# norlab-ulaval/norlab_icp_mapper

Hardware: AMD Instinct MI355X
Metric: ICP iterations/sec, 100k-pt scan vs 1M-pt map (higher is better)
Workload: dtype f32; 1 GPU; single synthetic 100000-pt scan vs 1000000-pt map, point-to-point ICP, KDTreeMatcher knn 1 maxDist 2.0 epsilon 0, TrimmedDist 0.85, fixed 20 iterations per registration; chain=p2p, scene=box+pillars sigma=0.01 seeds 42/43/44 (SURVEY.md 8d), parallelism=scan-sharded x1, map replicated

## Files before the change

### norlab_icp_mapper_amd/csrc/common.h

```cpp
#pragma once

#include <hip/hip_runtime.h>
#include <stdint.h>
#include <math.h>
#include <cstring>
#include <string>
#include <vector>
#include <unordered_map>
#include <mutex>
#include <map>
#include <cstdlib>
#include <shared_mutex>

#include "../../include/icpmi.h"

#define ICPMI_NV 32
#define ICPMI_MAX_OUTLIER 8
#define ICPMI_MAX_SMOOTH 16
#define ICPMI_SEL_BINS 2048
#ifndef ICPMI_S2_COPIES
#define ICPMI_S2_COPIES 8
#endif
#define ICPMI_S2_C0 4096
#define ICPMI_S2_F0 (ICPMI_S2_C0 + ICPMI_S2_COPIES * 256)
#ifndef ICPMI_S2_FCOPIES
#define ICPMI_S2_FCOPIES 1
#endif
#define ICPMI_S2_C1 (ICPMI_S2_F0 + ICPMI_S2_FCOPIES * 65536)
#define ICPMI_S2_F1 (ICPMI_S2_C1 + 256)
#define ICPMI_ACC_COPIES 2
#define ICPMI_ACC_MAX_ADDS 128
#define ICPMI_ACC_PAD 16
#define ICPMI_ACC_U64 (ICPMI_ACC_COPIES * ICPMI_NV * 2 * ICPMI_ACC_PAD)
#define ICPMI_ACC_IDX(copy, i, limb) ((((copy) * ICPMI_NV + (i)) * 2 + (limb)) * ICPMI_ACC_PAD)
#define ICPMI_ACC_FLAG (ICPMI_ACC_IDX(0, 0, 0) + 8)
#define ICPMI_S2_ACC (ICPMI_S2_F1 + 65536)
#define ICPMI_WIN_BINS 7
#ifndef ICPMI_WIN_COPIES
#define ICPMI_WIN_COPIES 8
#endif
#define ICPMI_WIN_PAD 16
#define ICPMI_WIN_HDR (ICPMI_WIN_COPIES * 3 * ICPMI_WIN_PAD)
#define ICPMI_WIN_U64 (ICPMI_WIN_HDR + ICPMI_WIN_PAD)
#define ICPMI_WIN_MAX_COUNT (1ll << 21)
#define ICPMI_S2_WIN (ICPMI_S2_ACC + 2 * ICPMI_ACC_U64)
#define ICPMI_SELHIST_WORDS (ICPMI_S2_WIN + 2 * ICPMI_WIN_U64)
#define ICPMI_S2_FIDX(b) ((((b) & 255u) << 8) | ((b) >> 8))

#define ICPMI_MAX_K 32

#ifdef __HIPCC__
typedef float icpmi_vf4 __attribute__((ext_vector_type(4)));
#ifdef ICPMI_NT_STREAMS
__device__ __forceinline__ float4 ld_stream(const float4* p) { const icpmi_vf4 v = __builtin_nontemporal_load(reinterpret_cast<const icpmi_vf4*>(p)); return make_float4(v.x, v.y, v.z, v.w); }
__device__ __forceinline__ float ld_stream(const float* p) { return __builtin_nontemporal_load(p); }
__device__ __forceinline__ int ld_stream(const int* p) { return __builtin_nontemporal_load(p); }
__device__ __forceinline__ void st_stream(float4* p, float4 v) { icpmi_vf4 w; w.x = v.x; w.y = v.y; w.z = v.z; w.w = v.w; __builtin_nontemporal_store(w, reinterpret_cast<icpmi_vf4*>(p)); }
__device__ __forceinline__ void st_stream(float* p, float v) { __builtin_nontemporal_store(v, p); }
__device__ __forceinline__ void st_stream(int* p, int v) { __builtin_nontemporal_store(v, p); }
#else
template <class T> __device__ __forceinline__ T ld_stream(const T* p) { return *p; }
template <class T> __device__ __forceinline__ void st_stream(T* p, T v) { *p = v; }
#endif

struct WaveRun { bool head; int rank; int len; int head_lane; };
__device__ __forceinline__ WaveRun wave_run(unsigned key, bool valid)
{
    const int lane = threadIdx.x & 63;
    const unsigned prev = (unsigned)__shfl_up((int)key, 1, 64);
    const bool pvalid = __shfl_up((int)valid, 1, 64) != 0;
    const bool head = valid && (lane == 0 || !pvalid || prev != key);
    const unsigned long long heads = __ballot(head);
    const unsigned long long valids = __ballot(valid);
    WaveRun r;
    r.head = head;
    const unsigned long long below = heads & ((lane == 63) ? ~0ull : ((2ull << lane) - 1ull));
    r.head_lane = below ? 63 - __clzll((long long)below) : lane;
    r.rank = lane - r.head_lane;
    const unsigned long long above = (lane == 63) ? 0ull : (heads & ~((2ull << lane) - 1ull));
// ... 25 lines not shown
struct BatchArgs {
    int nscan;
    int qstride;
    int n[ICPMI_MAX_BATCH];
};
struct BatchSrc { const float4* p[ICPMI_MAX_BATCH]; };
static inline BatchArgs batch_of_one(int64_t n) { BatchArgs b; memset(&b, 0, sizeof b); b.nscan = 1; b.n[0] = (int)n; return b; }

struct LoopCfg {
    int   k;
    float max_dist;
    float maxr2;
    float inv1e, err2;
    int   ring_max;
    int   minimizer;
    int   n_out;
    int   out_type[ICPMI_MAX_OUTLIER];
    float out_param[ICPMI_MAX_OUTLIER];
    int   out_iparam[ICPMI_MAX_OUTLIER];
    float out_param2[ICPMI_MAX_OUTLIER];
    float out_param3[ICPMI_MAX_OUTLIER];
    int   ext;
    int   force_4dof;
    int   force_2d;
    int   is_2d;
    int   max_iter;
    int   use_diff;
    float min_rot, min_trans;
    int   smooth;
    int   use_bound;
    float max_rot, max_trans;
    int   has_read_normals;
    int   sensor_noise;
    const float* read_scalar;
};

struct IcpState {
    float T_iter[16];
    int   iter;
    int   done;
    int   error;
    int   stop_reason;
    int   counter;
    int   hist_n;
    double hq[(ICPMI_MAX_SMOOTH + 1) * 4];
    double ht[(ICPMI_MAX_SMOOTH + 1) * 3];
    double hrot[ICPMI_MAX_SMOOTH + 1];
    double htr[ICPMI_MAX_SMOOTH + 1];
    double init_q[4];
    unsigned sel_prefix;
    unsigned sel_rank;
    unsigned n_valid;
    unsigned sel_prefix_l[3];
    unsigned sel_rank_l[3];
    float limits[ICPMI_MAX_OUTLIER];
    unsigned vt_valid;
    float vt_ratio;
    float robust_med;
    float robust_scale;
    long long pairs;
    double wsum;
    unsigned hard_count;
    unsigned ticket;
    unsigned long long hard_total;
    unsigned seq;
    unsigned long long dbg[24];
// ... 655 lines not shown
```

### norlab_icp_mapper_amd/csrc/loop.hip

```cpp
#include "common.h"
#include "solve.h"
#include <cstring>

namespace {

template <int PASS, int MODE = 0>
__global__ __launch_bounds__(256) void sel_hist_kernel(const float* __restrict__ d2, int64_t count,
                                                       const IcpState* __restrict__ st, unsigned* __restrict__ ghist, int nb_scale = 0)
{
    if (st->done) return;
    if (blockIdx.x == 0 && threadIdx.x == 0) nn_stamp_close(const_cast<IcpState*>(st));
    if (MODE != 0 && nb_scale != 0 && st->iter + 1 > nb_scale) return;
    if (MODE == 3 && st->iter != 0) return;
    __shared__ unsigned h[ICPMI_SEL_BINS];
    for (int b = threadIdx.x; b < ICPMI_SEL_BINS; b += 256) h[b] = 0;
    __syncthreads();
    const unsigned prefix = st->sel_prefix;
    const float med = MODE == 2 ? st->robust_med : 0.f;
    for (int64_t i = (int64_t)blockIdx.x * 256 + threadIdx.x; i < count; i += (int64_t)gridDim.x * 256) {
        float v = d2[i];
        if (MODE == 0 || MODE == 3) { if (!(v != INFINITY && v > 0.f)) continue; }
        else {
            if (v == INFINITY) continue;
            if (MODE == 2) v = fabsf(v - med);
// ... 505 lines not shown
                const float rz = fmaf(T[10], az, fmaf(T[6], ay, T[2] * ax));
                ax = rx; ay = ry; az = rz;
            }
            const float4 b = ref_normals[sidx];
            const float dot = fmaf(az, b.z, fmaf(ay, b.y, ax * b.x));
            w *= (dot > cosf(prm)) ? 1.f : 0.f;
        } else if (EXT && type == ICPMI_OUT_GENERICDESCRIPTOR) {
            const int ip = lc.out_iparam[f];
            const float v = (ip & ICPMI_GEN_SOURCE_READING) ? lc.read_scalar[qi] : ref_scalar[orig];
            w *= (ip & ICPMI_GEN_SOFT) ? v : ((ip & ICPMI_GEN_LARGER) ? (v > prm ? 1.f : 0.f) : (v < prm ? 1.f : 0.f));
        } else if (EXT && type == ICPMI_OUT_ROBUST) {
            const int ip = lc.out_iparam[f];
            const int se = (ip >> 4) & 15, fct = ip & 15;
            const float sc = se != ICPMI_SCALE_NONE ? st->robust_scale : 1.f;
            const float res = ((ip >> 8) & 15) == ICPMI_DIST_POINT2PLANE ? plane2 : d2;
            const float kk = se != ICPMI_SCALE_BERG ? prm : (fct == ICPMI_ROB_CAUCHY ? 4.3040f : fct == ICPMI_ROB_TUKEY ? 7.0589f : fct == ICPMI_ROB_HUBER ? 2.0138f : prm);
            const float e2 = res / (sc * sc);
            const float apx = lc.out_param3[f];
            float rw = robust_weight(fct, e2, kk);
            if (apx > 0.f && apx != INFINITY && e2 >= apx * apx) rw = 0.f;
            w *= rw;
        }
    }
    return w;
}

__host__ __device__ __forceinline__ int acc_threads(int k) { return k > 1 ? 1024 : 256; }
__host__ __device__ __forceinline__ int acc_blocks_dev(int64_t count, int cap, int bt = 256)
{
    const int64_t nb = (count + bt - 1) / bt;
    return (int)(nb < 1 ? 1 : (nb > cap ? cap : nb));
}

template <int MIN, bool FUSED, bool EXT, int BT = 256>
__global__ __launch_bounds__(BT) void accumulate_kernel(const float4* __restrict__ reading, BatchArgs ba, int acc_cap, LoopCfg lc,
                                                         IcpState* __restrict__ st, const float4* __restrict__ map,
                                                         const float4* __restrict__ normals,
                                                         const float4* __restrict__ read_normals,
                                                         const int* __restrict__ sidx, const float* __restrict__ d2a,
                                                         unsigned* __restrict__ hists,
                                                         int fused_slot, int is_median, float factor,
                                                         const float4* __restrict__ match_pt, const int* __restrict__ qindex,
                                                         const float* __restrict__ ref_scalar, const float4* __restrict__ pnm)
{
    const int n = ba.n[blockIdx.y];
    const int nbe = acc_blocks_dev((int64_t)n * lc.k, acc_cap, BT);
    if ((int)blockIdx.x >= nbe) return;
    {
        const size_t qo = (size_t)blockIdx.y * (size_t)ba.qstride;
        reading += qo; sidx += qo * lc.k; d2a += qo * lc.k;
        if (match_pt) match_pt += qo;
        if (qindex) qindex += qo;
        if (read_normals) read_normals += qo;
        hists += (size_t)blockIdx.y * ICPMI_SELHIST_WORDS;
        st += blockIdx.y;
    }
    const int64_t count = (int64_t)n * lc.k;
    const int64_t stride = (int64_t)nbe * BT;
    const int64_t gtid = (int64_t)blockIdx.x * BT + threadIdx.x;
#ifdef ICPMI_ACC_STRIDED
    const int64_t estep = stride;
    const int64_t e_first = gtid, e_end = count;
#else
    const int64_t estep = BT;
    const int wgc = (nbe & 7) == 0 ? (int)(blockIdx.x & 7) * (nbe >> 3) + (int)(blockIdx.x >> 3) : (int)blockIdx.x;
    const int64_t per_wg = (count + nbe - 1) / nbe;
    const int64_t e_first = (int64_t)wgc * per_wg + threadIdx.x;
    const int64_t e_end = ((int64_t)wgc + 1) * per_wg < count ? ((int64_t)wgc + 1) * per_wg : count;
#endif
    constexpr int PF = BT > 256 ? 3 : 2;
    float pd2[PF]; int ps[PF]; float4 pr[PF], pq[PF];
#pragma unroll
    for (int u = 0; u < PF; ++u) {
        const int64_t e = e_first + u * estep;
        const bool in = e < e_end;
        pd2[u] = in ? ld_stream(d2a + e) : INFINITY;
        ps[u] = in ? ld_stream(sidx + e) : -1;
        pr[u] = ld_stream(reading + (in ? (int)(e / lc.k) : 0));
        pq[u] = (match_pt && in) ? ld_stream(match_pt + e) : ((pnm && ps[u] >= 0) ? pnm[2 * (size_t)ps[u]] : make_float4(0.f, 0.f, 0.f, 0.f));
    }
    const unsigned cv = (FUSED && threadIdx.x < 256) ? hists[ICPMI_S2_C1 + threadIdx.x] : 0u;
    float4 pn[PF];
#pragma unroll
    for (int u = 0; u < PF; ++u)
        pn[u] = (MIN == ICPMI_MIN_POINT_TO_PLANE && ps[u] >= 0) ? (pnm ? pnm[2 * (size_t)ps[u] + 1] : normals[ps[u]]) : make_float4(0.f, 0.f, 0.f, 0.f);
    if (st->done) return;
    if (blockIdx.x == 0 && threadIdx.x == 0) nn_stamp_close(const_cast<IcpState*>(st));
    float fused_limit = 0.f;
    if (FUSED) {
        __shared__ unsigned shsel[16];
        unsigned bin, rem, total;
        block_find_rank_2tier<1>(cv, hists + ICPMI_S2_F1, false, 0.f, st->sel_rank_l[0], shsel, bin, rem, total);
        const float q = __uint_as_float((st->sel_prefix_l[0] << 16) | bin);
        fused_limit = is_median ? factor * q : q;
        if (blockIdx.x == 0 && threadIdx.x == 0) st->limits[fused_slot] = fused_limit;
        for (int64_t i = gtid; i < ICPMI_S2_COPIES * 256 + ICPMI_S2_FCOPIES * 65536; i += stride) hists[ICPMI_S2_C0 + i] = 0;
        if (lc.k > 1) for (int64_t i = gtid; i < 2 * ICPMI_WIN_U64; i += stride) hists[ICPMI_S2_WIN + i] = 0;
    }
    constexpr int NVAL = MIN == ICPMI_MIN_POINT_TO_PLANE ? 27 : (MIN == ICPMI_MIN_POINT_TO_POINT ? 16 : 0);
    double acc[NVAL > 0 ? NVAL : 1];
#pragma unroll
    for (int i = 0; i < (NVAL > 0 ? NVAL : 1); ++i) acc[i] = 0.0;
    double wsum = 0.0, cnt = 0.0;
    double b2d[3] = {0.0, 0.0, 0.0};
    const float* T = st->T_iter;
    auto pair = [&](int64_t e, float d2, int s, float4 r, float4 qkept, float4 nkept, bool have_n) {
        if (d2 == INFINITY) return;
        const int qi = (int)(e / lc.k);
        float w;
        if (EXT) {
            const float3 pe = xf_point(T, r.x, r.y, r.z, r.w);
            const float4 qe = (match_pt || (pnm && have_n)) ? qkept : (pnm ? pnm[2 * (size_t)s] : map[s]);
            float plane2 = 0.f;
            if (normals) {
                const float4 ne = have_n && MIN == ICPMI_MIN_POINT_TO_PLANE ? nkept : (pnm ? pnm[2 * (size_t)s + 1] : normals[s]);
                const float dx = pe.x - qe.x, dy = pe.y - qe.y, dz = pe.z - qe.z;
                const float dot = dx * ne.x + dy * ne.y + dz * ne.z;
                plane2 = dot * dot;
            }
            w = match_weight<true>(lc, st, d2, T, read_normals, qindex ? qindex[qi] : qi, normals, s, FUSED ? fused_slot : -1, fused_limit,
                                   ref_scalar, __float_as_int(qe.w), plane2);
        } else w = match_weight(lc, st, d2, T, read_normals, qindex ? qindex[qi] : qi, normals, s, FUSED ? fused_slot : -1, fused_limit);
        if (w == 0.f) return;
        wsum += w; cnt += 1.0;
        if (MIN == ICPMI_MIN_IDENTITY) return;
        const float3 p = xf_point(T, r.x, r.y, r.z, r.w);
        const float4 q = (match_pt || (pnm && have_n)) ? qkept : (pnm ? pnm[2 * (size_t)s] : map[s]);
        if (MIN == ICPMI_MIN_POINT_TO_POINT) {
// ... 36 lines not shown
    const int lane = threadIdx.x & 63, wv = threadIdx.x >> 6;
    double val[ICPMI_NV];
#pragma unroll
    for (int i = 0; i < ICPMI_NV; ++i) val[i] = i < NVAL ? acc[i < NVAL ? i : 0] : 0.0;
    val[27] = wsum; val[28] = cnt;
    if (EXT) { val[29] = b2d[0]; val[30] = b2d[1]; val[31] = b2d[2]; }
#pragma unroll
    for (int s = 0; s < 5; ++s) {
        const int m = 1 << s;
        const int nkeep = 16 >> s;
        const bool upper = (lane & m) != 0;
#pragma unroll
        for (int i = 0; i < nkeep; ++i) {
            const double send = upper ? val[i] : val[i + nkeep];
            const double keep = upper ? val[i + nkeep] : val[i];
            val[i] = keep + __shfl_xor(send, m, 64);
        }
    }
    val[0] += __shfl_xor(val[0], 32, 64);
    if (lane < 32) {
        const int idx = ((lane & 1) << 4) | ((lane & 2) << 2) | (lane & 4) | ((lane & 8) >> 2) | ((lane & 16) >> 4);
        sh[wv][idx] = val[0];
    }
    __syncthreads();
    if (threadIdx.x < ICPMI_NV) {
        const int i = threadIdx.x;
        double v = 0.0;
        if (i < NVAL || i == 27 || i == 28 || (EXT && i > 28)) {
            v = sh[0][i] + sh[1][i] + sh[2][i] + sh[3][i];
#pragma unroll
            for (int w2 = 4; w2 < BT / 64; ++w2) v += sh[w2][i];
        }
        unsigned long long* acc = reinterpret_cast<unsigned long long*>(hists + ICPMI_S2_ACC);
        if (v != 0.0) {
            if (!(fabs(v) < 0x1p77)) atomicOr(reinterpret_cast<unsigned*>(acc + ICPMI_ACC_FLAG), 1u);
            else {
                const double hi = rint(v * 0x1p-16);
                const double lo = v - hi * 65536.0;
                const long long H = (long long)hi, Lq = __double2ll_rn(lo * 0x1p40);
                const int cp = blockIdx.x & (ICPMI_ACC_COPIES - 1);
                if (H) atomicAdd(acc + ICPMI_ACC_IDX(cp, i, 0), (unsigned long long)H);
                if (Lq) atomicAdd(acc + ICPMI_ACC_IDX(cp, i, 1), (unsigned long long)Lq);
            }
        }
    }
}

__device__ __forceinline__ void mirror_state(const IcpState* st, IcpState* mirror)
{
    const unsigned* src = reinterpret_cast<const unsigned*>(st);
    unsigned* dst = reinterpret_cast<unsigned*>(mirror);
    constexpr int W = (int)(sizeof(IcpState) / sizeof(unsigned));
    for (int i = threadIdx.x; i < W; i += 64) dst[i] = __hip_atomic_load(src + i, __ATOMIC_RELAXED, __HIP_MEMORY_SCOPE_AGENT);
}

__global__ __launch_bounds__(256) void solve_kernel(IcpState* __restrict__ st, unsigned* __restrict__ hists, int clear, LoopCfg lc,
                                                    float* __restrict__ T_step_out, double* __restrict__ sums_out, unsigned* __restrict__ progress,
                                                    IcpState* __restrict__ mirror)
{
    st += blockIdx.x;
    unsigned long long* acc = reinterpret_cast<unsigned long long*>(hists + (size_t)blockIdx.x * ICPMI_SELHIST_WORDS + ICPMI_S2_ACC);
    if (progress) progress += blockIdx.x;
    if (threadIdx.x == 0 && st->hard_count) { st->hard_total += st->hard_count; st->hard_count = 0; }
    if (st->done) {
        if (mirror && threadIdx.x < 64) mirror_state(st, mirror + blockIdx.x);
        if (threadIdx.x == 0) publish_progress(st, progress);
        return;
    }
    solve_body(st, acc, clear != 0, lc, T_step_out, sums_out);
    if (threadIdx.x == 0 && st->done) st->t_done = (unsigned long long)wall_clock64();
    if (mirror) {
        __syncthreads();
        if (threadIdx.x < 64 && __hip_atomic_load(&st->done, __ATOMIC_RELAXED, __HIP_MEMORY_SCOPE_AGENT)) mirror_state(st, mirror + blockIdx.x);
    }
    if (threadIdx.x == 0) publish_progress(st, progress);
}

__global__ __launch_bounds__(256) void centre_kernel(BatchSrc src, BatchArgs ba, float mx, float my, float mz, float4* __restrict__ out)
{
    const int64_t n = ba.n[blockIdx.y];
    const float4* __restrict__ scan = src.p[blockIdx.y];
    out += (size_t)blockIdx.y * (size_t)ba.qstride;
    const int64_t i = (int64_t)blockIdx.x * 256 + threadIdx.x;
    if (i >= n) return;
    const float4 p = scan[i];
    out[i] = make_float4(fmaf(-mx, p.w, p.x), fmaf(-my, p.w, p.y), fmaf(-mz, p.w, p.z), p.w);
// ... 52 lines not shown
        const double e1 = 1.0 + (double)cfg.epsilon;
        lc.inv1e = (float)(1.0 / e1); if ((double)lc.inv1e < 1.0 / e1) lc.inv1e = nextafterf(lc.inv1e, 2.f);
        lc.err2 = (float)(e1 * e1); if ((double)lc.err2 > e1 * e1) lc.err2 = nextafterf(lc.err2, 0.f);
    }
    const int RING_CAP = 16;
    if (std::isfinite(cfg.max_dist) && c->grid.cell > 0.f) {
        const int need = (int)ceilf(cfg.max_dist / c->grid.cell) + 1;
        lc.ring_max = need < RING_CAP ? need : RING_CAP;
    } else lc.ring_max = 6;
    if (lc.ring_max < 1) lc.ring_max = 1;
    lc.minimizer = cfg.minimizer;
    lc.n_out = cfg.n_outlier;
    for (int f = 0; f < cfg.n_outlier && f < ICPMI_MAX_OUTLIER; ++f) {
        lc.out_type[f] = cfg.outlier[f].type;
        lc.out_param[f] = cfg.outlier[f].param;
        lc.out_iparam[f] = cfg.outlier[f].iparam;
        lc.out_param2[f] = cfg.outlier[f].param2;
        lc.out_param3[f] = cfg.outlier[f].param3;
        if (lc.out_type[f] == ICPMI_OUT_GENERICDESCRIPTOR || lc.out_type[f] == ICPMI_OUT_ROBUST) lc.ext = 1;
    }
    lc.force_4dof = cfg.force_4dof != 0 && cfg.minimizer == ICPMI_MIN_POINT_TO_PLANE;
    lc.is_2d = cfg.is_2d != 0;
    lc.force_2d = (cfg.force_2d != 0 || cfg.is_2d != 0) && cfg.minimizer == ICPMI_MIN_POINT_TO_PLANE;
    if (lc.force_2d) lc.ext = 1;
    if (fixed_iterations > 0) {
        lc.max_iter = fixed_iterations; lc.use_diff = 0; lc.use_bound = 0;
    } else {
        lc.max_iter = cfg.max_iterations;
        lc.use_diff = cfg.use_differential; lc.use_bound = cfg.use_bound;
    }
    lc.min_rot = cfg.min_diff_rot; lc.min_trans = cfg.min_diff_trans;
    lc.smooth = cfg.smooth_length < 1 ? 1 : (cfg.smooth_length > ICPMI_MAX_SMOOTH ? ICPMI_MAX_SMOOTH : cfg.smooth_length);
    lc.max_rot = cfg.max_rot_norm; lc.max_trans = cfg.max_trans_norm;
    return lc;
}

template <int MODE>
__global__ __launch_bounds__(256) void overlap_kernel(const float4* __restrict__ reading, const int* __restrict__ qindex, int n, LoopCfg lc,
                                                      const IcpState* __restrict__ st, const float4* __restrict__ map,
                                                      const float4* __restrict__ ref_normals, const float4* __restrict__ read_normals,
                                                      const float* __restrict__ noise, const int* __restrict__ sidx, const float* __restrict__ d2a,
                                                      const float4* __restrict__ match_pt, float mean, double* __restrict__ partial,
                                                      unsigned long long* __restrict__ count)
{
    const float* T = st->T_prev;
    const int64_t total = (int64_t)n * lc.k;
    double np = 0.0, sd = 0.0;
    unsigned long long cnt = 0;
    for (int64_t e = (int64_t)blockIdx.x * 256 + threadIdx.x; e < total; e += (int64_t)gridDim.x * 256) {
        const float d2 = d2a[e];
        if (d2 == INFINITY) continue;
        const int qi = (int)(e / lc.k);
        const int oi = qindex ? qindex[qi] : qi;
        const int s = sidx[e];
        const float w = match_weight(lc, st, d2, T, read_normals, oi, ref_normals, s);
        if (w == 0.f) continue;
        const float4 r = reading[qi];
        const float3 p = xf_point(T, r.x, r.y, r.z, r.w);
        const float4 q = match_pt ? match_pt[e] : map[s];
        const float dx = p.x - q.x, dy = p.y - q.y, dz = p.z - q.z;
        if (lc.minimizer == ICPMI_MIN_POINT_TO_POINT) {
            const float dist = sqrtf(fmaf(dz, dz, fmaf(dy, dy, dx * dx)));
            if (MODE == 0) { np += 1.0; sd += (double)dist; }
            else if (dist < mean + noise[oi]) ++cnt;
        } else {
            const float4 a = read_normals[oi];
// ... 387 lines not shown
                           (const long long*)vb.best_idx, vb.nchunks, min_el, f);
    }
    if (slot >= 0) {
        const float quant = lc.out_type[slot] == ICPMI_OUT_MEDIANDIST ? 0.5f : lc.out_param[slot];
        const BatchArgs ba = cur_batch(c, count / lc.k);
        if (!c->nn_builds_hist0)
        {
            int hb0 = (int)std::min<int64_t>((count + 4095) / 4096, 256);
            if (hb0 < 1) hb0 = 1;
            hipLaunchKernelGGL(sel2_hist0_kernel, dim3(hb0, ba.nscan), dim3(256), 0, c->stream, c->d_d2, ba, lc.k, c->d_state, c->d_selhist, quant,
                               c->nn_builds_win ? 1 : 0);
        }
        int hb2 = (int)std::min<int64_t>((count + 511) / 512, 512);
        if (hb2 < 1) hb2 = 1;
        hipLaunchKernelGGL(sel2_scan_hist_kernel, dim3(hb2, ba.nscan), dim3(256), 0, c->stream, c->d_d2, ba, lc.k, c->d_state, c->d_selhist, quant,
                           (c->nn_builds_win && !c->nn_builds_hist0) ? 1 : 0);
        return;
    }
    for (int f = 0; f < lc.n_out; ++f) {
        const int type = lc.out_type[f];
        if (type != ICPMI_OUT_TRIMMEDDIST && type != ICPMI_OUT_MEDIANDIST) continue;
        const int is_med = type == ICPMI_OUT_MEDIANDIST;
        const float quant = is_med ? 0.5f : lc.out_param[f];
        const float factor = lc.out_param[f];
        hipLaunchKernelGGL((sel_hist_kernel<0, 0>), dim3(hb), dim3(256), 0, c->stream, c->d_d2, count, c->d_state, c->d_selhist, 0);
        hipLaunchKernelGGL(sel_scan_kernel<0>, dim3(1), dim3(256), 0, c->stream, c->d_state, c->d_selhist, quant, f, is_med, factor, 0, 0);
        hipLaunchKernelGGL((sel_hist_kernel<1, 0>), dim3(hb), dim3(256), 0, c->stream, c->d_d2, count, c->d_state, c->d_selhist, 0);
        hipLaunchKernelGGL(sel_scan_kernel<1>, dim3(1), dim3(256), 0, c->stream, c->d_state, c->d_selhist, quant, f, is_med, factor, 0, 0);
        hipLaunchKernelGGL((sel_hist_kernel<2, 0>), dim3(hb), dim3(256), 0, c->stream, c->d_d2, count, c->d_state, c->d_selhist, 0);
        hipLaunchKernelGGL(sel_scan_kernel<2>, dim3(1), dim3(256), 0, c->stream, c->d_state, c->d_selhist, quant, f, is_med, factor, 0, 0);
    }
}

template <int MIN, bool FUSED, bool EXT>
static void launch_accumulate_ext(icpmi_ctx* c, int64_t n, const LoopCfg& lc, int nb, int slot);

template <int MIN, bool FUSED>
static void launch_accumulate(icpmi_ctx* c, int64_t n, const LoopCfg& lc, int nb, int slot)
{
    if (lc.ext) launch_accumulate_ext<MIN, FUSED, true>(c, n, lc, nb, slot);
    else launch_accumulate_ext<MIN, FUSED, false>(c, n, lc, nb, slot);
}

template <int MIN, bool FUSED, bool EXT>
static void launch_accumulate_ext(icpmi_ctx* c, int64_t n, const LoopCfg& lc, int nb, int slot)
{
    const float4* rn = lc.has_read_normals ? c->d_read_normals : nullptr;
    const int is_med = slot >= 0 && lc.out_type[slot] == ICPMI_OUT_MEDIANDIST;
    const float factor = slot >= 0 ? lc.out_param[slot] : 0.f;
    const bool sorted = c->nn_out_sorted;
    const BatchArgs ba = cur_batch(c, n);
    if (lc.k > 1) {
        hipLaunchKernelGGL((accumulate_kernel<MIN, FUSED, EXT, 1024>), dim3(nb, ba.nscan), dim3(1024), 0, c->stream, sorted ? c->d_qsorted : c->d_reading, ba, acc_cap(), lc, c->d_state,
                           c->d_map_sorted, c->has_normals ? c->d_normals_sorted : (const float4*)nullptr, rn, c->d_sidx, c->d_d2, c->d_selhist, slot, is_med, factor,
                           (const float4*)nullptr, sorted ? c->d_qindex : (const int*)nullptr, (EXT && c->raw_has_scalar) ? c->d_raw_s : (const float*)nullptr,
                           (MIN == ICPMI_MIN_POINT_TO_PLANE && c->has_normals && c->d_map_pn) ? c->d_map_pn : (const float4*)nullptr);
        return;
    }
    hipLaunchKernelGGL((accumulate_kernel<MIN, FUSED, EXT>), dim3(nb, ba.nscan), dim3(256), 0, c->stream, sorted ? c->d_qsorted : c->d_reading, ba, acc_cap(), lc, c->d_state,
                       c->d_map_sorted, c->has_normals ? c->d_normals_sorted : (const float4*)nullptr, rn, c->d_sidx, c->d_d2, c->d_selhist, slot, is_med, factor,
                       (sorted && lc.k == 1) ? c->d_match_pt : (const float4*)nullptr, sorted ? c->d_qindex : (const int*)nullptr,
                       (EXT && c->raw_has_scalar) ? c->d_raw_s : (const float*)nullptr,
                       (lc.k > 1 && MIN == ICPMI_MIN_POINT_TO_PLANE && c->has_normals && c->d_map_pn) ? c->d_map_pn : (const float4*)nullptr);
}

static void enqueue_accumulate_solve(icpmi_ctx* c, int64_t n, const LoopCfg& lc, float* d_Tstep, double* d_sums)
{
    const int64_t count = n * lc.k;
    const int nb = acc_blocks(count, acc_threads(lc.k));
    const int slot = fused_filter_slot(lc);
    const bool fused = slot >= 0;
    if (lc.minimizer == ICPMI_MIN_POINT_TO_PLANE) {
        if (fused) launch_accumulate<ICPMI_MIN_POINT_TO_PLANE, true>(c, n, lc, nb, slot);
        else launch_accumulate<ICPMI_MIN_POINT_TO_PLANE, false>(c, n, lc, nb, slot);
    } else if (lc.minimizer == ICPMI_MIN_POINT_TO_POINT) {
        if (fused) launch_accumulate<ICPMI_MIN_POINT_TO_POINT, true>(c, n, lc, nb, slot);
        else launch_accumulate<ICPMI_MIN_POINT_TO_POINT, false>(c, n, lc, nb, slot);
    } else {
        if (fused) launch_accumulate<ICPMI_MIN_IDENTITY, true>(c, n, lc, nb, slot);
        else launch_accumulate<ICPMI_MIN_IDENTITY, false>(c, n, lc, nb, slot);
    }
    const BatchArgs ba = cur_batch(c, n);
    hipLaunchKernelGGL(solve_kernel, dim3(ba.nscan), dim3(256), 0, c->stream, c->d_state, c->d_selhist, 1, lc, d_Tstep, d_sums,
                       c->d_progress, ba.nscan == 1 ? c->d_state_mirror : (IcpState*)nullptr);
}

static icpmi_status enqueue_iteration(icpmi_ctx* c, int64_t n, const LoopCfg& lc, hipEvent_t nn0, hipEvent_t nn1)
{
    if (nn0) HIP_TRY(c, hipEventRecord(nn0, c->stream));
    c->nn_hist0 = fused_filter_slot(lc) >= 0 ? c->d_selhist : nullptr;
    c->nn_builds_hist0 = false;
    c->nn_builds_win = false;
    c->nn_match_pt = lc.k == 1 ? c->d_match_pt : nullptr;
    c->nn_sorted_k = lc.k > 1;
    c->nn_out_sorted = false;
    icpmi_status s = nn_launch_k(c, c->d_reading, n, c->d_state->T_iter, lc, 1, c->d_sidx, c->d_d2, c->d_state);
    c->nn_sorted_k = false;
    if (s != ICPMI_OK) return s;
    if (nn1) HIP_TRY(c, hipEventRecord(nn1, c->stream));
    enqueue_selection(c, lc, n * lc.k);
    enqueue_accumulate_solve(c, n, lc, nullptr, nullptr);
    HIP_TRY(c, hipGetLastError());
    return ICPMI_OK;
}

static void fill_stats(const IcpState* hs, const LoopCfg& lc, int64_t n, icpmi_stats* stats, bool with_dbg = true)
{
    if (!stats) return;
    stats->iterations = hs->iter;
    stats->stop_reason = hs->stop_reason;
    stats->pairs = hs->pairs;
    const double denom = (double)lc.k * (double)n;
    stats->point_used_ratio = denom > 0 ? (float)hs->pairs / (float)denom : 0.f;
    stats->weighted_point_used_ratio = denom > 0 ? (float)(hs->wsum / denom) : 0.f;
// ... 498 lines not shown
```

### norlab_icp_mapper_amd/csrc/solve.h

```cpp
#pragma once
#include "common.h"

namespace {

__device__ void mat4_mul_dev(const float* A, const float* B, float* C)
{
    float R[16];
#pragma unroll
    for (int j = 0; j < 4; ++j)
#pragma unroll
        for (int i = 0; i < 4; ++i) {
            float s = A[i] * B[4 * j];
#pragma unroll
            for (int kk = 1; kk < 4; ++kk) s = fmaf(A[4 * kk + i], B[4 * j + kk], s);
            R[4 * j + i] = s;
        }
#pragma unroll
    for (int i = 0; i < 16; ++i) C[i] = R[i];
}

__device__ void jacobi_eig(int n, const double* Ain, double* w, double* Q)
{
    __shared__ double A[36];
    for (int i = 0; i < n * n; ++i) A[i] = Ain[i];
// ... 336 lines not shown
        s = fmaf(nrm * z, ps, nrm);
        float pc = fmaf(z, -2.75573192e-07f, 2.48015873e-05f);
        pc = fmaf(z, pc, -1.38888889e-03f);
        pc = fmaf(z, pc, 4.16666667e-02f);
        pc = fmaf(z, pc, -0.5f);
        c = fmaf(z, pc, 1.f);
    } else { s = (float)sin((double)nrm); c = (float)cos((double)nrm); }
    const float sx = s * ax, sy = s * ay, sz = s * az;
    const float cx = (1.f - c) * ax, cy = (1.f - c) * ay, cz = (1.f - c) * az;
    float tmp;
    tmp = cx * ay; T[4 * 1 + 0] = tmp - sz; T[4 * 0 + 1] = tmp + sz;
    tmp = cx * az; T[4 * 2 + 0] = tmp + sy; T[4 * 0 + 2] = tmp - sy;
    tmp = cy * az; T[4 * 2 + 1] = tmp - sx; T[4 * 1 + 2] = tmp + sx;
    T[0] = cx * ax + c; T[5] = cy * ay + c; T[10] = cz * az + c;
}

__device__ double quat_angdist(const double* a, const double* b)
{
    const double w = a[0] * b[0] + a[1] * b[1] + a[2] * b[2] + a[3] * b[3];
    const double x = -a[0] * b[1] + a[1] * b[0] - a[2] * b[3] + a[3] * b[2];
    const double y = -a[0] * b[2] + a[1] * b[3] + a[2] * b[0] - a[3] * b[1];
    const double z = -a[0] * b[3] - a[1] * b[2] + a[2] * b[1] + a[3] * b[0];
    return 2.0 * atan2(sqrt(x * x + y * y + z * z), fabs(w));
}

__device__ __forceinline__ unsigned pair_sum_mask(const LoopCfg& lc)
{
    const unsigned nval = lc.minimizer == ICPMI_MIN_POINT_TO_PLANE ? 27u : (lc.minimizer == ICPMI_MIN_POINT_TO_POINT ? 16u : 0u);
    unsigned m = (nval ? ((1u << nval) - 1u) : 0u) | (1u << 27) | (1u << 28);
    if (lc.force_2d) m |= 7u << 29;
    return m;
}

__device__ __forceinline__ void read_pair_sums(unsigned long long* __restrict__ acc, double* __restrict__ tot , bool clear, bool* nonfinite,
                                               unsigned mask = 0xffffffffu)
{
    __shared__ long long ph[ICPMI_ACC_COPIES][ICPMI_NV], pl[ICPMI_ACC_COPIES][ICPMI_NV];
    __shared__ unsigned s_flag;
    const int t = threadIdx.x;
    if (t < ICPMI_ACC_COPIES * ICPMI_NV) {
        const int i = t & (ICPMI_NV - 1), cp = t >> 5;
        unsigned long long a = 0ull, b = 0ull;
        if ((mask >> i) & 1u) { a = acc[ICPMI_ACC_IDX(cp, i, 0)]; b = acc[ICPMI_ACC_IDX(cp, i, 1)]; }
        ph[cp][i] = (long long)a; pl[cp][i] = (long long)b;
        if (clear) { if (a) acc[ICPMI_ACC_IDX(cp, i, 0)] = 0ull; if (b) acc[ICPMI_ACC_IDX(cp, i, 1)] = 0ull; }
    }
    if (t == ICPMI_ACC_COPIES * ICPMI_NV) {
        unsigned* fl = reinterpret_cast<unsigned*>(acc + ICPMI_ACC_FLAG);
        s_flag = *fl;
        if (clear && s_flag) *fl = 0u;
    }
    __syncthreads();
    if (t < ICPMI_NV) {
        long long H = 0, Lq = 0;
#pragma unroll
        for (int cp = 0; cp < ICPMI_ACC_COPIES; ++cp) { H += ph[cp][t]; Lq += pl[cp][t]; }
        tot[t] = (double)H * 65536.0 + (double)Lq * 0x1p-40;
    }
    __syncthreads();
    *nonfinite = s_flag != 0u;
}

__device__ void solve_serial(IcpState* st, const double* tot, const LoopCfg& lc, float* T_step_out)
{
    const long long tsolve0 = clock64();

    const double wsum = tot[27];
    const long long P = (long long)(tot[28] + 0.5);
    st->pairs = P;
    st->wsum = wsum;
    if (P == 0) { st->error = ICPMI_ERR_NO_POINT_TO_MINIMIZE; st->done = 1; return; }

    float Ts[16];
    for (int i = 0; i < 16; ++i) Ts[i] = (i % 5 == 0) ? 1.f : 0.f;
    if (lc.minimizer == ICPMI_MIN_POINT_TO_POINT) {
        const double iw = 1.0 / wsum;
        const double mpd[3] = {tot[1] * iw, tot[2] * iw, tot[3] * iw}, mqd[3] = {tot[4] * iw, tot[5] * iw, tot[6] * iw};
        __shared__ float H[9];
        for (int c = 0; c < 3; ++c)
            for (int r = 0; r < 3; ++r) H[3 * c + r] = (float)(tot[7 + 3 * c + r] - mqd[r] * tot[1 + c]);
        __shared__ float R[9];
        if (lc.is_2d) {
            const float a = H[0] + H[4], b2 = H[1] - H[3];
// ... 66 lines not shown
                         dz = st->ht[3 * a + 2] - st->ht[3 * bq + 2];
            st->htr[a] = sqrt(dx * dx + dy * dy + dz * dz);
        }
        if (hn > SL) {
            double rot = 0, tr = 0;
            for (int i = hn - 1; i >= hn - SL; --i) { rot += st->hrot[i % RING]; tr += st->htr[i % RING]; }
            rot /= SL; tr /= SL;
            if (rot != rot || tr != tr) { st->error = ICPMI_ERR_NAN; st->done = 1; return; }
            if (rot < (double)lc.min_rot && tr < (double)lc.min_trans) {
                if (iterate) reason = ICPMI_STOP_DIFFERENTIAL;
                iterate = false;
            }
        }
    }
    if (lc.use_bound) {
        __shared__ double q[4];
        quat_from_T(Ti, q);
        const double rot = fabs(quat_angdist(q, st->init_q));
        const double nt = sqrt((double)Ti[12] * Ti[12] + (double)Ti[13] * Ti[13] + (double)Ti[14] * Ti[14]);
        if (rot > (double)lc.max_rot || nt > (double)lc.max_trans) { st->error = ICPMI_ERR_BOUND; st->done = 1; return; }
    }
    if (!iterate) { st->done = 1; st->stop_reason = reason; }
    const long long tsolve3 = clock64();
#ifndef ICPMI_NN_TIMING
    st->dbg[20] += (unsigned long long)(tsolve3 - tsolve0);
    st->dbg[21] += 1;
    st->dbg[22] += (unsigned long long)(tsolve1 - tsolve0);
    st->dbg[23] += (unsigned long long)(tsolve3 - tsolve2);
#else
    (void)tsolve1; (void)tsolve2; (void)tsolve3;
#endif
}

__device__ void solve_body(IcpState* __restrict__ st, unsigned long long* __restrict__ acc, bool clear, const LoopCfg& lc,
                           float* __restrict__ T_step_out, double* __restrict__ sums_out)
{
    __shared__ double tot[ICPMI_NV];
    const int t = threadIdx.x;
    bool nonfinite = false;
    read_pair_sums(acc, tot, clear, &nonfinite, pair_sum_mask(lc));
    if (t < ICPMI_NV && sums_out) sums_out[t] = tot[t];
    if (nonfinite) { if (t == 0) { st->error = ICPMI_ERR_NAN; st->done = 1; } return; }
    if (t == 0) solve_serial(st, tot, lc, T_step_out);
}

__device__ __forceinline__ void publish_progress(const IcpState* st, unsigned* progress)
{
    if (!progress) return;
    const unsigned v = ((unsigned)(st->done != 0) << 31) | ((st->seq & 0x7ffffu) << 12) | ((unsigned)st->iter & 0xfffu);
    __hip_atomic_store(progress, v, __ATOMIC_RELEASE, __HIP_MEMORY_SCOPE_SYSTEM);
}
struct ProgressWord { bool mine, done; int iter; };
static inline ProgressWord decode_progress(unsigned v, unsigned seq) { return {((v >> 12) & 0x7ffffu) == seq, (v >> 31) != 0, (int)(v & 0xfffu)}; }


}
```

Baseline: 23750 iterations/s.

## Fuse ICP solve into accumulate kernel via last-block ticket

Adds a TAIL variant of the fused accumulate kernel in which the last block to finish, chosen by an atomic ticket counter, runs the 6-DOF solve, mirrors the state and publishes progress. This removes the separate solve_kernel launch per iteration for k=1 trimmed-distance chains. Accumulator reads switch to coherent atomic loads so the last block sees every other block's sums. The cost is an extra atomic and two barriers per block, plus a serial solve inside the tail block.

```diff
diff --git a/norlab_icp_mapper_amd/csrc/common.h b/norlab_icp_mapper_amd/csrc/common.h
--- a/norlab_icp_mapper_amd/csrc/common.h
+++ b/norlab_icp_mapper_amd/csrc/common.h
@@ -44,7 +44,8 @@
 #define ICPMI_WIN_U64 (ICPMI_WIN_HDR + ICPMI_WIN_PAD)
 #define ICPMI_WIN_MAX_COUNT (1ll << 21)
 #define ICPMI_S2_WIN (ICPMI_S2_ACC + 2 * ICPMI_ACC_U64)
-#define ICPMI_SELHIST_WORDS (ICPMI_S2_WIN + 2 * ICPMI_WIN_U64)
+#define ICPMI_S2_TICKET (ICPMI_S2_WIN + 2 * ICPMI_WIN_U64)
+#define ICPMI_SELHIST_WORDS (ICPMI_S2_TICKET + 32)
 #define ICPMI_S2_FIDX(b) ((((b) & 255u) << 8) | ((b) >> 8))
 
 #define ICPMI_MAX_K 32
@@ -136,6 +137,7 @@
     float max_rot, max_trans;
     int   has_read_normals;
     int   sensor_noise;
+    int   tail_solve;
     const float* read_scalar;
 };
 
diff --git a/norlab_icp_mapper_amd/csrc/loop.hip b/norlab_icp_mapper_amd/csrc/loop.hip
--- a/norlab_icp_mapper_amd/csrc/loop.hip
+++ b/norlab_icp_mapper_amd/csrc/loop.hip
@@ -561,7 +561,15 @@
     return (int)(nb < 1 ? 1 : (nb > cap ? cap : nb));
 }
 
-template <int MIN, bool FUSED, bool EXT, int BT = 256>
+__device__ __forceinline__ void mirror_state(const IcpState* st, IcpState* mirror)
+{
+    const unsigned* src = reinterpret_cast<const unsigned*>(st);
+    unsigned* dst = reinterpret_cast<unsigned*>(mirror);
+    constexpr int W = (int)(sizeof(IcpState) / sizeof(unsigned));
+    for (int i = threadIdx.x; i < W; i += 64) dst[i] = __hip_atomic_load(src + i, __ATOMIC_RELAXED, __HIP_MEMORY_SCOPE_AGENT);
+}
+
+template <int MIN, bool FUSED, bool EXT, int BT = 256, bool TAIL = false>
 __global__ __launch_bounds__(BT) void accumulate_kernel(const float4* __restrict__ reading, BatchArgs ba, int acc_cap, LoopCfg lc,
                                                          IcpState* __restrict__ st, const float4* __restrict__ map,
                                                          const float4* __restrict__ normals,
@@ -570,8 +578,10 @@
                                                          unsigned* __restrict__ hists,
                                                          int fused_slot, int is_median, float factor,
                                                          const float4* __restrict__ match_pt, const int* __restrict__ qindex,
-                                                         const float* __restrict__ ref_scalar, const float4* __restrict__ pnm)
-{
+                                                         const float* __restrict__ ref_scalar, const float4* __restrict__ pnm,
+                                                         unsigned* __restrict__ progress, IcpState* __restrict__ mirror)
+{
+    static_assert(!TAIL || (FUSED && !EXT && BT == 256), "the solving variant serves the fused k = 1 chains");
     const int n = ba.n[blockIdx.y];
     const int nbe = acc_blocks_dev((int64_t)n * lc.k, acc_cap, BT);
     if ((int)blockIdx.x >= nbe) return;
@@ -583,6 +593,8 @@
         if (read_normals) read_normals += qo;
         hists += (size_t)blockIdx.y * ICPMI_SELHIST_WORDS;
         st += blockIdx.y;
+        if (TAIL && progress) progress += blockIdx.y;
+        if (TAIL && mirror) mirror += blockIdx.y;
     }
     const int64_t count = (int64_t)n * lc.k;
     const int64_t stride = (int64_t)nbe * BT;
@@ -613,8 +625,15 @@
 #pragma unroll
     for (int u = 0; u < PF; ++u)
         pn[u] = (MIN == ICPMI_MIN_POINT_TO_PLANE && ps[u] >= 0) ? (pnm ? pnm[2 * (size_t)ps[u] + 1] : normals[ps[u]]) : make_float4(0.f, 0.f, 0.f, 0.f);
-    if (st->done) return;
-    if (blockIdx.x == 0 && threadIdx.x == 0) nn_stamp_close(const_cast<IcpState*>(st));
+    if (st->done) {
+        if (TAIL && blockIdx.x == 0) {
+            if (threadIdx.x == 0 && st->hard_count) { st->hard_total += st->hard_count; st->hard_count = 0; }
+            if (mirror && threadIdx.x < 64) mirror_state(st, mirror);
+            if (threadIdx.x == 0) publish_progress(st, progress);
+        }
+        return;
+    }
+    if (!TAIL && blockIdx.x == 0 && threadIdx.x == 0) nn_stamp_close(const_cast<IcpState*>(st));
     float fused_limit = 0.f;
     if (FUSED) {
         __shared__ unsigned shsel[16];
@@ -622,7 +641,7 @@
         block_find_rank_2tier<1>(cv, hists + ICPMI_S2_F1, false, 0.f, st->sel_rank_l[0], shsel, bin, rem, total);
         const float q = __uint_as_float((st->sel_prefix_l[0] << 16) | bin);
         fused_limit = is_median ? factor * q : q;
-        if (blockIdx.x == 0 && threadIdx.x == 0) st->limits[fused_slot] = fused_limit;
+        if (!TAIL && blockIdx.x == 0 && threadIdx.x == 0) st->limits[fused_slot] = fused_limit;
         for (int64_t i = gtid; i < ICPMI_S2_COPIES * 256 + ICPMI_S2_FCOPIES * 65536; i += stride) hists[ICPMI_S2_C0 + i] = 0;
         if (lc.k > 1) for (int64_t i = gtid; i < 2 * ICPMI_WIN_U64; i += stride) hists[ICPMI_S2_WIN + i] = 0;
     }
@@ -725,26 +744,43 @@
             for (int w2 = 4; w2 < BT / 64; ++w2) v += sh[w2][i];
         }
         unsigned long long* acc = reinterpret_cast<unsigned long long*>(hists + ICPMI_S2_ACC);
+        unsigned long long old = 0ull;
         if (v != 0.0) {
-            if (!(fabs(v) < 0x1p77)) atomicOr(reinterpret_cast<unsigned*>(acc + ICPMI_ACC_FLAG), 1u);
+            if (!(fabs(v) < 0x1p77)) old |= atomicOr(reinterpret_cast<unsigned*>(acc + ICPMI_ACC_FLAG), 1u);
             else {
                 const double hi = rint(v * 0x1p-16);
                 const double lo = v - hi * 65536.0;
                 const long long H = (long long)hi, Lq = __double2ll_rn(lo * 0x1p40);
                 const int cp = blockIdx.x & (ICPMI_ACC_COPIES - 1);
-                if (H) atomicAdd(acc + ICPMI_ACC_IDX(cp, i, 0), (unsigned long long)H);
-                if (Lq) atomicAdd(acc + ICPMI_ACC_IDX(cp, i, 1), (unsigned long long)Lq);
+                if (H) old |= atomicAdd(acc + ICPMI_ACC_IDX(cp, i, 0), (unsigned long long)H);
+                if (Lq) old |= atomicAdd(acc + ICPMI_ACC_IDX(cp, i, 1), (unsigned long long)Lq);
             }
         }
-    }
-}
-
-__device__ __forceinline__ void mirror_state(const IcpState* st, IcpState* mirror)
-{
-    const unsigned* src = reinterpret_cast<const unsigned*>(st);
-    unsigned* dst = reinterpret_cast<unsigned*>(mirror);
-    constexpr int W = (int)(sizeof(IcpState) / sizeof(unsigned));
-    for (int i = threadIdx.x; i < W; i += 64) dst[i] = __hip_atomic_load(src + i, __ATOMIC_RELAXED, __HIP_MEMORY_SCOPE_AGENT);
+        if (TAIL) asm volatile("" :: "v"((unsigned)old), "v"((unsigned)(old >> 32)));
+    }
+    if (TAIL) {
+        __shared__ unsigned s_last;
+        unsigned* ticket = hists + ICPMI_S2_TICKET;
+        __syncthreads();
+        if (threadIdx.x == 0) s_last = __hip_atomic_fetch_add(ticket, 1u, __ATOMIC_RELAXED, __HIP_MEMORY_SCOPE_AGENT) == (unsigned)nbe - 1u ? 1u : 0u;
+        __syncthreads();
+        if (!s_last) return;
+        if (threadIdx.x == 0) {
+            __hip_atomic_store(ticket, 0u, __ATOMIC_RELAXED, __HIP_MEMORY_SCOPE_AGENT);
+            if (st->hard_count) { st->hard_total += st->hard_count; st->hard_count = 0; }
+            st->limits[fused_slot] = fused_limit;
+#ifndef ICPMI_NN_TIMING
+            st->dbg[10] += 1ull;
+#endif
+        }
+        solve_body<true>(st, reinterpret_cast<unsigned long long*>(hists + ICPMI_S2_ACC), true, lc, nullptr, nullptr);
+        if (threadIdx.x == 0 && st->done) st->t_done = (unsigned long long)wall_clock64();
+        if (mirror) {
+            __syncthreads();
+            if (threadIdx.x < 64 && __hip_atomic_load(&st->done, __ATOMIC_RELAXED, __HIP_MEMORY_SCOPE_AGENT)) mirror_state(st, mirror);
+        }
+        if (threadIdx.x == 0) publish_progress(st, progress);
+    }
 }
 
 __global__ __launch_bounds__(256) void solve_kernel(IcpState* __restrict__ st, unsigned* __restrict__ hists, int clear, LoopCfg lc,
@@ -863,6 +899,17 @@
     lc.min_rot = cfg.min_diff_rot; lc.min_trans = cfg.min_diff_trans;
     lc.smooth = cfg.smooth_length < 1 ? 1 : (cfg.smooth_length > ICPMI_MAX_SMOOTH ? ICPMI_MAX_SMOOTH : cfg.smooth_length);
     lc.max_rot = cfg.max_rot_norm; lc.max_trans = cfg.max_trans_norm;
+    {
+        int nq = 0, trimmed = 0;
+        for (int f = 0; f < lc.n_out; ++f) {
+            nq += lc.out_type[f] == ICPMI_OUT_TRIMMEDDIST || lc.out_type[f] == ICPMI_OUT_MEDIANDIST;
+            trimmed += lc.out_type[f] == ICPMI_OUT_TRIMMEDDIST;
+        }
+        const bool minimises = lc.minimizer == ICPMI_MIN_POINT_TO_POINT || lc.minimizer == ICPMI_MIN_POINT_TO_PLANE;
+        const char* e = getenv("ICPMI_TAIL_SOLVE");
+        const bool off = e && atoi(e) == 0;
+        lc.tail_solve = !off && lc.k == 1 && nq == 1 && trimmed == 1 && !lc.ext && minimises;
+    }
     return lc;
 }
 
@@ -1316,17 +1363,18 @@
     }
 }
 
-template <int MIN, bool FUSED, bool EXT>
+template <int MIN, bool FUSED, bool EXT, bool TAIL = false>
 static void launch_accumulate_ext(icpmi_ctx* c, int64_t n, const LoopCfg& lc, int nb, int slot);
 
 template <int MIN, bool FUSED>
-static void launch_accumulate(icpmi_ctx* c, int64_t n, const LoopCfg& lc, int nb, int slot)
+static void launch_accumulate(icpmi_ctx* c, int64_t n, const LoopCfg& lc, int nb, int slot, bool tail)
 {
     if (lc.ext) launch_accumulate_ext<MIN, FUSED, true>(c, n, lc, nb, slot);
+    else if (FUSED && MIN != ICPMI_MIN_IDENTITY && tail) launch_accumulate_ext<MIN, FUSED, false, FUSED && MIN != ICPMI_MIN_IDENTITY>(c, n, lc, nb, slot);
     else launch_accumulate_ext<MIN, FUSED, false>(c, n, lc, nb, slot);
 }
 
-template <int MIN, bool FUSED, bool EXT>
+template <int MIN, bool FUSED, bool EXT, bool TAIL>
 static void launch_accumulate_ext(icpmi_ctx* c, int64_t n, const LoopCfg& lc, int nb, int slot)
 {
     const float4* rn = lc.has_read_normals ? c->d_read_normals : nullptr;
@@ -1338,14 +1386,16 @@
         hipLaunchKernelGGL((accumulate_kernel<MIN, FUSED, EXT, 1024>), dim3(nb, ba.nscan), dim3(1024), 0, c->stream, sorted ? c->d_qsorted : c->d_reading, ba, acc_cap(), lc, c->d_state,
                            c->d_map_sorted, c->has_normals ? c->d_normals_sorted : (const float4*)nullptr, rn, c->d_sidx, c->d_d2, c->d_selhist, slot, is_med, factor,
                            (const float4*)nullptr, sorted ? c->d_qindex : (const int*)nullptr, (EXT && c->raw_has_scalar) ? c->d_raw_s : (const float*)nullptr,
-                           (MIN == ICPMI_MIN_POINT_TO_PLANE && c->has_normals && c->d_map_pn) ? c->d_map_pn : (const float4*)nullptr);
+                           (MIN == ICPMI_MIN_POINT_TO_PLANE && c->has_normals && c->d_map_pn) ? c->d_map_pn : (const float4*)nullptr,
+                           (unsigned*)nullptr, (IcpState*)nullptr);
         return;
     }
-    hipLaunchKernelGGL((accumulate_kernel<MIN, FUSED, EXT>), dim3(nb, ba.nscan), dim3(256), 0, c->stream, sorted ? c->d_qsorted : c->d_reading, ba, acc_cap(), lc, c->d_state,
+    hipLaunchKernelGGL((accumulate_kernel<MIN, FUSED, EXT, 256, TAIL>), dim3(nb, ba.nscan), dim3(256), 0, c->stream, sorted ? c->d_qsorted : c->d_reading, ba, acc_cap(), lc, c->d_state,
                        c->d_map_sorted, c->has_normals ? c->d_normals_sorted : (const float4*)nullptr, rn, c->d_sidx, c->d_d2, c->d_selhist, slot, is_med, factor,
                        (sorted && lc.k == 1) ? c->d_match_pt : (const float4*)nullptr, sorted ? c->d_qindex : (const int*)nullptr,
                        (EXT && c->raw_has_scalar) ? c->d_raw_s : (const float*)nullptr,
-                       (lc.k > 1 && MIN == ICPMI_MIN_POINT_TO_PLANE && c->has_normals && c->d_map_pn) ? c->d_map_pn : (const float4*)nullptr);
+                       (lc.k > 1 && MIN == ICPMI_MIN_POINT_TO_PLANE && c->has_normals && c->d_map_pn) ? c->d_map_pn : (const float4*)nullptr,
+                       TAIL ? c->d_progress : (unsigned*)nullptr, (TAIL && ba.nscan == 1) ? c->d_state_mirror : (IcpState*)nullptr);
 }
 
 static void enqueue_accumulate_solve(icpmi_ctx* c, int64_t n, const LoopCfg& lc, float* d_Tstep, double* d_sums)
@@ -1354,16 +1404,18 @@
     const int nb = acc_blocks(count, acc_threads(lc.k));
     const int slot = fused_filter_slot(lc);
     const bool fused = slot >= 0;
+    const bool tail = lc.tail_solve && fused && !d_Tstep && !d_sums;
     if (lc.minimizer == ICPMI_MIN_POINT_TO_PLANE) {
-        if (fused) launch_accumulate<ICPMI_MIN_POINT_TO_PLANE, true>(c, n, lc, nb, slot);
-        else launch_accumulate<ICPMI_MIN_POINT_TO_PLANE, false>(c, n, lc, nb, slot);
+        if (fused) launch_accumulate<ICPMI_MIN_POINT_TO_PLANE, true>(c, n, lc, nb, slot, tail);
+        else launch_accumulate<ICPMI_MIN_POINT_TO_PLANE, false>(c, n, lc, nb, slot, false);
     } else if (lc.minimizer == ICPMI_MIN_POINT_TO_POINT) {
-        if (fused) launch_accumulate<ICPMI_MIN_POINT_TO_POINT, true>(c, n, lc, nb, slot);
-        else launch_accumulate<ICPMI_MIN_POINT_TO_POINT, false>(c, n, lc, nb, slot);
+        if (fused) launch_accumulate<ICPMI_MIN_POINT_TO_POINT, true>(c, n, lc, nb, slot, tail);
+        else launch_accumulate<ICPMI_MIN_POINT_TO_POINT, false>(c, n, lc, nb, slot, false);
     } else {
-        if (fused) launch_accumulate<ICPMI_MIN_IDENTITY, true>(c, n, lc, nb, slot);
-        else launch_accumulate<ICPMI_MIN_IDENTITY, false>(c, n, lc, nb, slot);
-    }
+        if (fused) launch_accumulate<ICPMI_MIN_IDENTITY, true>(c, n, lc, nb, slot, tail);
+        else launch_accumulate<ICPMI_MIN_IDENTITY, false>(c, n, lc, nb, slot, false);
+    }
+    if (tail) return;
     const BatchArgs ba = cur_batch(c, n);
     hipLaunchKernelGGL(solve_kernel, dim3(ba.nscan), dim3(256), 0, c->stream, c->d_state, c->d_selhist, 1, lc, d_Tstep, d_sums,
                        c->d_progress, ba.nscan == 1 ? c->d_state_mirror : (IcpState*)nullptr);
diff --git a/norlab_icp_mapper_amd/csrc/solve.h b/norlab_icp_mapper_amd/csrc/solve.h
--- a/norlab_icp_mapper_amd/csrc/solve.h
+++ b/norlab_icp_mapper_amd/csrc/solve.h
@@ -392,23 +392,26 @@
     return m;
 }
 
+template <bool COHERENT = false>
 __device__ __forceinline__ void read_pair_sums(unsigned long long* __restrict__ acc, double* __restrict__ tot , bool clear, bool* nonfinite,
                                                unsigned mask = 0xffffffffu)
 {
+    auto ld = [](const auto* p) { return COHERENT ? __hip_atomic_load(p, __ATOMIC_RELAXED, __HIP_MEMORY_SCOPE_AGENT) : *p; };
+    auto zero = [](auto* p) { if (COHERENT) __hip_atomic_store(p, decltype(*p + 0)(0), __ATOMIC_RELAXED, __HIP_MEMORY_SCOPE_AGENT); else *p = 0; };
     __shared__ long long ph[ICPMI_ACC_COPIES][ICPMI_NV], pl[ICPMI_ACC_COPIES][ICPMI_NV];
     __shared__ unsigned s_flag;
     const int t = threadIdx.x;
     if (t < ICPMI_ACC_COPIES * ICPMI_NV) {
         const int i = t & (ICPMI_NV - 1), cp = t >> 5;
         unsigned long long a = 0ull, b = 0ull;
-        if ((mask >> i) & 1u) { a = acc[ICPMI_ACC_IDX(cp, i, 0)]; b = acc[ICPMI_ACC_IDX(cp, i, 1)]; }
+        if ((mask >> i) & 1u) { a = ld(acc + ICPMI_ACC_IDX(cp, i, 0)); b = ld(acc + ICPMI_ACC_IDX(cp, i, 1)); }
         ph[cp][i] = (long long)a; pl[cp][i] = (long long)b;
-        if (clear) { if (a) acc[ICPMI_ACC_IDX(cp, i, 0)] = 0ull; if (b) acc[ICPMI_ACC_IDX(cp, i, 1)] = 0ull; }
+        if (clear) { if (a) zero(acc + ICPMI_ACC_IDX(cp, i, 0)); if (b) zero(acc + ICPMI_ACC_IDX(cp, i, 1)); }
     }
     if (t == ICPMI_ACC_COPIES * ICPMI_NV) {
         unsigned* fl = reinterpret_cast<unsigned*>(acc + ICPMI_ACC_FLAG);
-        s_flag = *fl;
-        if (clear && s_flag) *fl = 0u;
+        s_flag = ld(fl);
+        if (clear && s_flag) zero(fl);
     }
     __syncthreads();
     if (t < ICPMI_NV) {
@@ -541,13 +544,14 @@
 #endif
 }
 
+template <bool COHERENT = false>
 __device__ void solve_body(IcpState* __restrict__ st, unsigned long long* __restrict__ acc, bool clear, const LoopCfg& lc,
                            float* __restrict__ T_step_out, double* __restrict__ sums_out)
 {
     __shared__ double tot[ICPMI_NV];
     const int t = threadIdx.x;
     bool nonfinite = false;
-    read_pair_sums(acc, tot, clear, &nonfinite, pair_sum_mask(lc));
+    read_pair_sums<COHERENT>(acc, tot, clear, &nonfinite, pair_sum_mask(lc));
     if (t < ICPMI_NV && sums_out) sums_out[t] = tot[t];
     if (nonfinite) { if (t == 0) { st->error = ICPMI_ERR_NAN; st->done = 1; } return; }
     if (t == 0) solve_serial(st, tot, lc, T_step_out);
```

After: 23320 iterations/s. 1.8% lower.
